# microsoft/XPretrain

Measured on NVIDIA H100. Metric: video-text pairs/sec (12f x 224^2, 32 tok), CLIP-ViP ViT-B/16 fwd+InfoNCE+bwd, higher is better.
Workload: dtype bf16

## Files before the change

### xpretrain_b200/csrc/common.cu

```cuda
#include "common.h"

#include <mutex>

#include "../../include/xpretrain_b200.h"

namespace xp {

static thread_local std::string t_error;
std::atomic<int64_t> g_launches{0};

void set_error(const std::string& msg) { t_error = msg; }
int fail(const std::string& msg) {
  t_error = msg;
  return -1;
}

int sm_count() {
  static int cached[64] = {0};
  int dev = 0;
  if (cudaGetDevice(&dev) != cudaSuccess || dev < 0 || dev >= 64) return 132;
  if (cached[dev] == 0) {
    int n = 0;
    if (cudaDeviceGetAttribute(&n, cudaDevAttrMultiProcessorCount, dev) != cudaSuccess || n <= 0) n = 132;
    cached[dev] = n;
  }
  return cached[dev];
}

typedef CUresult (*EncodeTiledFn)(CUtensorMap*, CUtensorMapDataType, cuuint32_t, void*, const cuuint64_t*,
                                  const cuuint64_t*, const cuuint32_t*, const cuuint32_t*, CUtensorMapInterleave,
                                  CUtensorMapSwizzle, CUtensorMapL2promotion, CUtensorMapFloatOOBfill);

static EncodeTiledFn encode_fn() {
  static EncodeTiledFn fn = nullptr;
  static std::once_flag once;
  std::call_once(once, [] {
    void* p = nullptr;
    cudaDriverEntryPointQueryResult q;
    if (cudaGetDriverEntryPoint("cuTensorMapEncodeTiled", &p, cudaEnableDefault, &q) == cudaSuccess &&
        q == cudaDriverEntryPointSuccess)
      fn = reinterpret_cast<EncodeTiledFn>(p);
  });
  return fn;
}

typedef CUresult (*CtxGetCurrentFn)(CUcontext*);
typedef CUresult (*CtxSetCurrentFn)(CUcontext);
typedef CUresult (*PointerGetAttributeFn)(void*, CUpointer_attribute, CUdeviceptr);

static void* driver_symbol(const char* name) {
  void* p = nullptr;
  cudaDriverEntryPointQueryResult q;
  if (cudaGetDriverEntryPoint(name, &p, cudaEnableDefault, &q) != cudaSuccess || q != cudaDriverEntryPointSuccess)
    return nullptr;
  return p;
}

int ensure_context(const void* device_ptr) {
  static thread_local bool bound = false;
  if (bound) return 0;
  static CtxGetCurrentFn get_cur = reinterpret_cast<CtxGetCurrentFn>(driver_symbol("cuCtxGetCurrent"));
  static CtxSetCurrentFn set_cur = reinterpret_cast<CtxSetCurrentFn>(driver_symbol("cuCtxSetCurrent"));
  static PointerGetAttributeFn ptr_attr =
      reinterpret_cast<PointerGetAttributeFn>(driver_symbol("cuPointerGetAttribute"));
  if (!get_cur || !set_cur || !ptr_attr)
    return fail("CUDA driver unavailable (no GPU): this library has no CPU path");
  CUcontext cur = nullptr;
  if (get_cur(&cur) == CUDA_SUCCESS && cur != nullptr) {
    bound = true;
    return 0;
  }
  if (device_ptr == nullptr) return fail("null device pointer");
  CUcontext owner = nullptr;
  if (ptr_attr(&owner, CU_POINTER_ATTRIBUTE_CONTEXT, reinterpret_cast<CUdeviceptr>(device_ptr)) == CUDA_SUCCESS &&
      owner != nullptr) {
    if (set_cur(owner) != CUDA_SUCCESS) return fail("cuCtxSetCurrent failed");
  } else {
    int ordinal = -1;
    if (ptr_attr(&ordinal, CU_POINTER_ATTRIBUTE_DEVICE_ORDINAL, reinterpret_cast<CUdeviceptr>(device_ptr)) !=
            CUDA_SUCCESS ||
        ordinal < 0)
      return fail("cannot find the CUDA device of the first pointer argument (is it a device pointer?)");
    if (cudaSetDevice(ordinal) != cudaSuccess) return fail("cudaSetDevice failed");
  }
  bound = true;
  return 0;
}

int make_tmap_bf16_2d(CUtensorMap* out, const void* base, uint64_t inner, uint64_t outer, uint64_t row_stride,
                      uint32_t box_inner, uint32_t box_outer) {
  EncodeTiledFn fn = encode_fn();
  if (!fn) return fail("cuTensorMapEncodeTiled unavailable (no CUDA driver / no GPU): this library has no CPU path");
  if ((reinterpret_cast<uintptr_t>(base) & 15) != 0) return fail("tensor map: base pointer must be 16-byte aligned");
  if ((row_stride * 2) % 16 != 0) return fail("tensor map: row stride must be a multiple of 8 bf16 elements");
  cuuint64_t dims[2] = {inner, outer};
  cuuint64_t strides[1] = {row_stride * 2};
  cuuint32_t box[2] = {box_inner, box_outer};
  cuuint32_t estr[2] = {1, 1};
  CUresult r = fn(out, CU_TENSOR_MAP_DATA_TYPE_BFLOAT16, 2, const_cast<void*>(base), dims, strides, box, estr,
                  CU_TENSOR_MAP_INTERLEAVE_NONE, CU_TENSOR_MAP_SWIZZLE_128B, CU_TENSOR_MAP_L2_PROMOTION_L2_256B,
                  CU_TENSOR_MAP_FLOAT_OOB_FILL_NONE);
  if (r != CUDA_SUCCESS) return fail("cuTensorMapEncodeTiled failed with CUresult " + std::to_string(int(r)));
  return 0;
}

int make_tmap_bf16_3d(CUtensorMap* out, const void* base, uint64_t inner, uint64_t mid, uint64_t outer,
                      uint64_t row_stride, uint64_t mid_stride, uint32_t box_inner, uint32_t box_mid) {
  EncodeTiledFn fn = encode_fn();
  if (!fn) return fail("cuTensorMapEncodeTiled unavailable (no CUDA driver / no GPU): this library has no CPU path");
  if ((reinterpret_cast<uintptr_t>(base) & 15) != 0) return fail("tensor map: base pointer must be 16-byte aligned");
  if ((row_stride * 2) % 16 != 0 || (mid_stride * 2) % 16 != 0)
    return fail("tensor map: strides must be multiples of 8 bf16 elements");
  cuuint64_t dims[3] = {inner, mid, outer};
  cuuint64_t strides[2] = {row_stride * 2, mid_stride * 2};
  cuuint32_t box[3] = {box_inner, box_mid, 1};
  cuuint32_t estr[3] = {1, 1, 1};
  CUresult r = fn(out, CU_TENSOR_MAP_DATA_TYPE_BFLOAT16, 3, const_cast<void*>(base), dims, strides, box, estr,
                  CU_TENSOR_MAP_INTERLEAVE_NONE, CU_TENSOR_MAP_SWIZZLE_128B, CU_TENSOR_MAP_L2_PROMOTION_L2_256B,
                  CU_TENSOR_MAP_FLOAT_OOB_FILL_NONE);
  if (r != CUDA_SUCCESS) return fail("cuTensorMapEncodeTiled failed with CUresult " + std::to_string(int(r)));
  return 0;
}

}

extern "C" {
int xp_version(void) { return XP_ABI_VERSION; }
const char* xp_last_error(void) { return xp::t_error.c_str(); }
int64_t xp_launch_count(void) { return xp::g_launches.load(); }
void xp_launch_count_reset(void) { xp::g_launches.store(0); }
}
```

### xpretrain_b200/csrc/common.h

```cpp
#pragma once
#include <cuda.h>
#include <cuda_runtime.h>
#include <stdint.h>

#include <atomic>
#include <string>

namespace xp {

void set_error(const std::string& msg);
int fail(const std::string& msg);
extern std::atomic<int64_t> g_launches;
inline void count_launch(int n = 1) { g_launches.fetch_add(n, std::memory_order_relaxed); }

int sm_count();

int make_tmap_bf16_2d(CUtensorMap* out, const void* base, uint64_t inner, uint64_t outer, uint64_t row_stride,
                      uint32_t box_inner, uint32_t box_outer);
int make_tmap_bf16_3d(CUtensorMap* out, const void* base, uint64_t inner, uint64_t mid, uint64_t outer,
                      uint64_t row_stride, uint64_t mid_stride, uint32_t box_inner, uint32_t box_mid);

int ensure_context(const void* device_ptr);
#define XP_ENTER(ptr)                                   \
  do {                                                  \
    if (::xp::ensure_context(ptr) != 0) return -1;      \
  } while (0)

#define XP_CHECK_CUDA(expr)                                                                         \
  do {                                                                                              \
    cudaError_t _e = (expr);                                                                        \
    if (_e != cudaSuccess) return ::xp::fail(std::string(#expr) + ": " + cudaGetErrorString(_e)); \
  } while (0)

#define XP_CHECK_LAUNCH(name)                                                                             \
  do {                                                                                                    \
    cudaError_t _e = cudaGetLastError();                                                                  \
    if (_e != cudaSuccess) return ::xp::fail(std::string(name) + " launch: " + cudaGetErrorString(_e)); \
    ::xp::count_launch();                                                                                 \
  } while (0)

}
```

### xpretrain_b200/csrc/gemm.cu

```cuda
#include "../../include/xpretrain_b200.h"
#include "common.h"
#include "ptx.cuh"
#include <cstdlib>

namespace xp {

constexpr int BM = 128;
constexpr int BK = 64;
constexpr int MMA_K = 16;
constexpr int GEMM_THREADS = 384;

struct GemmDev {
  void* c;
  const float* bias;
  const __nv_bfloat16* residual;
  __nv_bfloat16* aux;
  int M, N, K;
  long long ldc, ldr, ld_aux;
  long long c_group, c_group_stride, r_group, r_group_stride;
  int act;
  int splits;
  int scale_cols;
  float alpha, col_scale;
  uint32_t mn_lbo, mn_sbo;
};

template <int BN>
struct GemmCfg {
  static constexpr int A_BYTES = BM * BK * 2;
  static constexpr int B_BYTES = BN * BK * 2;
  static constexpr int STAGE_BYTES = A_BYTES + B_BYTES;
  static constexpr int STAGES = (BN == 256) ? 4 : 6;
  static constexpr int SMEM_BYTES = STAGES * STAGE_BYTES + 1024 + 256;
};

__device__ __forceinline__ float act_gelu_erf(float x) { return 0.5f * x * (1.f + erff(x * 0.70710678118654752f)); }
__device__ __forceinline__ float act_gelu_erf_grad(float x) {
  float cdf = 0.5f * (1.f + erff(x * 0.70710678118654752f));
  float pdf = 0.3989422804014327f * __expf(-0.5f * x * x);
  return cdf + x * pdf;
}

template <int BN, int A_MN, int B_MN, int OUT, int ACT>
__global__ void __launch_bounds__(GEMM_THREADS, 1)
gemm_kernel(const __grid_constant__ CUtensorMap tmA, const __grid_constant__ CUtensorMap tmB, const GemmDev p) {
  using Cfg = GemmCfg<BN>;
  constexpr int STAGES = Cfg::STAGES;
  constexpr bool PINGPONG = BN == 128;
  constexpr int MH = PINGPONG ? 2 : 1;
  constexpr int NH = BN / 128;
  extern __shared__ uint8_t smem_raw[];
  const uint32_t raw_addr = smem_u32(smem_raw);
  uint8_t* smem = smem_raw + (((raw_addr + 1023u) & ~1023u) - raw_addr);
  uint64_t* full_bar = reinterpret_cast<uint64_t*>(smem + STAGES * Cfg::STAGE_BYTES);
  uint64_t* empty_bar = full_bar + STAGES;

  const int wg = threadIdx.x >> 7;
  const int lane = threadIdx.x & 31;

  const int num_m = (p.M + BM - 1) / BM;
  const int num_n = (p.N + BN - 1) / BN;
  const int num_mn = num_m * num_n;
  const int total = num_mn * p.splits;
  const int kb_total = (p.K + BK - 1) / BK;
  const int kb_per = (kb_total + p.splits - 1) / p.splits;

  if (threadIdx.x == 0) {
    tma_prefetch_desc(&tmA);
    tma_prefetch_desc(&tmB);
    for (int s = 0; s < STAGES; ++s) {
      mbar_init(&full_bar[s], 1);
      mbar_init(&empty_bar[s], PINGPONG ? 1 : 2);
    }
    fence_barrier_init();
  }
  __syncthreads();

  if (wg == 0) {
    setmaxnreg_dec<40>();
    if (threadIdx.x == 0) {
      int stage = 0;
      uint32_t phase = 0;
      for (int tile = blockIdx.x; tile < total; tile += gridDim.x) {
        const int split = tile / num_mn;
        const int mn = tile - split * num_mn;
        const int m_blk = mn / num_n;
        const int n_blk = mn - m_blk * num_n;
        const int k0 = split * kb_per;
        const int k1 = min(kb_total, k0 + kb_per);
        for (int kb = k0; kb < k1; ++kb) {
          mbar_wait_nocall(&empty_bar[stage], phase ^ 1);
          uint8_t* sA = smem + stage * Cfg::STAGE_BYTES;
          uint8_t* sB = sA + Cfg::A_BYTES;
          mbar_arrive_expect_tx(&full_bar[stage], Cfg::STAGE_BYTES);
          if (A_MN) {
#pragma unroll
            for (int i = 0; i < BM / 64; ++i)
              tma_load_2d(sA + i * (BK * 128), &tmA, &full_bar[stage], m_blk * BM + i * 64, kb * BK);
          } else {
            tma_load_2d(sA, &tmA, &full_bar[stage], kb * BK, m_blk * BM);
          }
          if (B_MN) {
#pragma unroll
            for (int i = 0; i < BN / 64; ++i)
              tma_load_2d(sB + i * (BK * 128), &tmB, &full_bar[stage], n_blk * BN + i * 64, kb * BK);
          } else {
            tma_load_2d(sB, &tmB, &full_bar[stage], kb * BK, n_blk * BN);
          }
          if (++stage == STAGES) {
            stage = 0;
            phase ^= 1;
          }
        }
      }
    }
  } else {
    setmaxnreg_inc<232>();
    const int cw = wg - 1;
    const int wq = (threadIdx.x >> 5) & 3;
    constexpr int act = ACT;
    const int N = p.N, scale_cols = p.scale_cols;
    const float alpha = p.alpha, col_scale = p.col_scale;
    __nv_bfloat16* const aux_p = p.aux;
    constexpr bool need_aux_in = (ACT == XP_ACT_DQUICK_GELU || ACT == XP_ACT_DGELU_ERF);
    const __nv_bfloat16* const xin_p = need_aux_in ? p.aux : p.residual;
    constexpr uint32_t A_OFF = 64 * 128;
    const int cta_tiles = (total - blockIdx.x + gridDim.x - 1) / gridDim.x;
    int stage = 0;
    uint32_t phase = 0;
    int local = 0;
    for (int tile = blockIdx.x; tile < total; tile += gridDim.x, ++local) {
      const int split = tile / num_mn;
      const int mn = tile - split * num_mn;
      const int m_blk = mn / num_n;
      const int n_blk = mn - m_blk * num_n;
      const int k0 = split * kb_per;
      const int k1 = min(kb_total, k0 + kb_per);
      if (PINGPONG && (local & 1) != cw) {
        const int next = stage + max(0, k1 - k0);
        phase ^= (next / STAGES) & 1;
        stage = next % STAGES;
        continue;
      }
      if (PINGPONG && local > 0) named_bar_sync(1 + cw, 256);
      const bool pass_turn = PINGPONG && local + 1 < cta_tiles;
      if (k0 >= k1) {
        if (pass_turn) named_bar_arrive(2 - cw, 256);
        continue;
      }
      float acc[MH * NH][64];
#pragma unroll
      for (int q = 0; q < MH * NH; ++q)
#pragma unroll
        for (int i = 0; i < 64; ++i) acc[q][i] = 0.f;
      int prev_stage = -1;
      for (int kb = k0; kb < k1; ++kb) {
        mbar_wait_nocall(&full_bar[stage], phase);
        const uint32_t sA = smem_u32(smem + stage * Cfg::STAGE_BYTES) + (PINGPONG ? 0 : cw * A_OFF);
        const uint32_t sB = smem_u32(smem + stage * Cfg::STAGE_BYTES) + Cfg::A_BYTES;
#pragma unroll
        for (int q = 0; q < MH * NH; ++q) wgmma_fence_regs(acc[q]);
        wgmma_fence();
#pragma unroll
        for (int j = 0; j < BK / MMA_K; ++j) {
#pragma unroll
          for (int mh = 0; mh < MH; ++mh) {
            const uint32_t am = sA + mh * A_OFF;
            const uint64_t adesc = A_MN ? make_smem_desc_sw128(am + j * (MMA_K * 128), p.mn_lbo, p.mn_sbo)
                                        : make_smem_desc_sw128(am + j * (MMA_K * 2), 16, 1024);
#pragma unroll
            for (int h = 0; h < NH; ++h) {
              const uint32_t bh = sB + h * (128 * 128);
              const uint64_t bdesc = B_MN ? make_smem_desc_sw128(bh + j * (MMA_K * 128), p.mn_lbo, p.mn_sbo)
                                          : make_smem_desc_sw128(bh + j * (MMA_K * 2), 16, 1024);
              wgmma_m64n128k16_bf16<A_MN, B_MN>(acc[mh * NH + h], adesc, bdesc);
            }
          }
        }
        wgmma_commit();
#pragma unroll
        for (int q = 0; q < MH * NH; ++q) wgmma_fence_regs(acc[q]);
        wgmma_wait<1>();
        if (prev_stage >= 0 && (threadIdx.x & 127) == 0) mbar_arrive(&empty_bar[prev_stage]);
        prev_stage = stage;
        if (++stage == STAGES) {
          stage = 0;
          phase ^= 1;
        }
      }
      if (pass_turn) named_bar_arrive(2 - cw, 256);
      const auto load_bias = [&](float2(&b)[16], int h) {
#pragma unroll
        for (int i = 0; i < 16; ++i) {
          const int n = n_blk * BN + h * 128 + i * 8 + (lane & 3) * 2;
          b[i] = make_float2(0.f, 0.f);
          if (p.bias != nullptr && split == 0 && n < N) b[i] = __ldg(reinterpret_cast<const float2*>(p.bias + n));
        }
      };
      constexpr bool bias_once = PINGPONG && !need_aux_in;
      float2 bias_tile[16];
      if (bias_once) load_bias(bias_tile, 0);
      wgmma_wait<0>();
#pragma unroll
      for (int q = 0; q < MH * NH; ++q) wgmma_fence_regs(acc[q]);
      if ((threadIdx.x & 127) == 0) mbar_arrive(&empty_bar[prev_stage]);

      const auto apply = [&](float& v0, float& v1, int n, uint32_t xg) -> uint32_t {
        if (n < scale_cols) {
          v0 *= col_scale;
          v1 *= col_scale;
        }
        uint32_t pre = 0;
        if (act == XP_ACT_QUICK_GELU) {
          pre = pack_bf16(v0, v1);
          v0 = quick_gelu(v0);
          v1 = quick_gelu(v1);
        } else if (act == XP_ACT_DQUICK_GELU) {
          v0 *= quick_gelu_grad(bf16_lo(xg));
          v1 *= quick_gelu_grad(bf16_hi(xg));
        } else if (act == XP_ACT_GELU_ERF) {
          pre = pack_bf16(v0, v1);
          v0 = act_gelu_erf(v0);
          v1 = act_gelu_erf(v1);
        } else if (act == XP_ACT_DGELU_ERF) {
          v0 *= act_gelu_erf_grad(bf16_lo(xg));
          v1 *= act_gelu_erf_grad(bf16_hi(xg));
        } else if (xin_p != nullptr) {
          v0 += bf16_lo(xg);
          v1 += bf16_hi(xg);
        }
        return pre;
      };
      constexpr bool save_pre = (ACT == XP_ACT_QUICK_GELU || ACT == XP_ACT_GELU_ERF);
      const int quad = lane & 3;
#pragma unroll
      for (int mh = 0; mh < MH; ++mh) {
        const int row_base = m_blk * BM + (PINGPONG ? mh : cw) * 64 + wq * 16 + (lane >> 2);
#pragma unroll
        for (int rr = 0; rr < 2; ++rr) {
          const int row = row_base + rr * 8;
          const bool row_ok = row < p.M;
          const long long c_off = p.c_group > 0 ? (row / p.c_group) * p.c_group_stride + (row % p.c_group) * p.ldc
                                                : static_cast<long long>(row) * p.ldc;
          const long long x_off = need_aux_in ? static_cast<long long>(row) * p.ld_aux
                                              : (p.r_group > 0 ? (row / p.r_group) * p.r_group_stride + (row % p.r_group) * p.ldr
                                                               : static_cast<long long>(row) * p.ldr);
          const long long a_off = static_cast<long long>(row) * p.ld_aux;
#pragma unroll
          for (int h = 0; h < NH; ++h) {
            const float* const a = acc[mh * NH + h];
            const int n_h = n_blk * BN + h * 128;
            float2 bias2[16];
            if (bias_once) {
#pragma unroll
              for (int i = 0; i < 16; ++i) bias2[i] = bias_tile[i];
            } else {
              load_bias(bias2, h);
            }
            if (OUT == XP_OUT_BF16) {
              uint32_t xin[4][4];
#pragma unroll
              for (int k = 0; k < 4; ++k) {
                const int n8 = n_h + (4 * k + quad) * 8;
                uint4 v = make_uint4(0u, 0u, 0u, 0u);
                if (xin_p != nullptr && row_ok && n8 < N) v = *reinterpret_cast<const uint4*>(xin_p + x_off + n8);
                xin[k][0] = v.x;
                xin[k][1] = v.y;
                xin[k][2] = v.z;
                xin[k][3] = v.w;
                if (xin_p != nullptr) quad_transpose(xin[k]);
              }
#pragma unroll
              for (int k = 0; k < 4; ++k) {
                uint32_t out[4], pre[4];
#pragma unroll
                for (int j = 0; j < 4; ++j) {
                  const int i = 4 * k + j;
                  float v0 = fmaf(a[4 * i + 2 * rr], alpha, bias2[i].x);
                  float v1 = fmaf(a[4 * i + 2 * rr + 1], alpha, bias2[i].y);
                  pre[j] = apply(v0, v1, n_h + i * 8 + quad * 2, xin[k][j]);
                  out[j] = pack_bf16(v0, v1);
                }
                const int n8 = n_h + (4 * k + quad) * 8;
                quad_transpose(out);
                if (row_ok && n8 < N)
                  *reinterpret_cast<uint4*>(static_cast<__nv_bfloat16*>(p.c) + c_off + n8) =
                      make_uint4(out[0], out[1], out[2], out[3]);
                if (save_pre && aux_p != nullptr) {
                  quad_transpose(pre);
                  if (row_ok && n8 < N)
                    *reinterpret_cast<uint4*>(aux_p + a_off + n8) = make_uint4(pre[0], pre[1], pre[2], pre[3]);
                }
              }
            } else if (row_ok) {
              uint32_t xin[16];
#pragma unroll
              for (int i = 0; i < 16; ++i) {
                const int n = n_h + i * 8 + quad * 2;
                xin[i] = 0;
                if (xin_p != nullptr && n < N) xin[i] = *reinterpret_cast<const uint32_t*>(xin_p + x_off + n);
              }
#pragma unroll
              for (int i = 0; i < 16; ++i) {
                const int n = n_h + i * 8 + quad * 2;
                if (n >= N) continue;
                float v0 = fmaf(a[4 * i + 2 * rr], alpha, bias2[i].x);
                float v1 = fmaf(a[4 * i + 2 * rr + 1], alpha, bias2[i].y);
                apply(v0, v1, n, xin[i]);
                if (OUT == XP_OUT_F32) {
                  *reinterpret_cast<float2*>(static_cast<float*>(p.c) + c_off + n) = make_float2(v0, v1);
                } else {
                  asm volatile("red.global.add.v2.f32 [%0], {%1, %2};" ::"l"(static_cast<float*>(p.c) + c_off + n),
                               "f"(v0), "f"(v1)
                               : "memory");
                }
              }
            }
          }
        }
      }
    }
  }
}

template <int BN, int A_MN, int B_MN, int OUT, int ACT>
static int launch_gemm(const CUtensorMap& tmA, const CUtensorMap& tmB, const GemmDev& dev, int grid, cudaStream_t stream) {
  using Cfg = GemmCfg<BN>;
  auto kern = gemm_kernel<BN, A_MN, B_MN, OUT, ACT>;
  static bool attr_set = false;
  if (!attr_set) {
    XP_CHECK_CUDA(cudaFuncSetAttribute(kern, cudaFuncAttributeMaxDynamicSharedMemorySize, Cfg::SMEM_BYTES));
    attr_set = true;
  }
  kern<<<grid, GEMM_THREADS, Cfg::SMEM_BYTES, stream>>>(tmA, tmB, dev);
  XP_CHECK_LAUNCH("gemm_kernel");
  return 0;
}

template <int BN, int OUT, int ACT>
static int dispatch_layout(const XpGemm* g, const CUtensorMap& tmA, const CUtensorMap& tmB, const GemmDev& dev,
                           int grid, cudaStream_t stream) {
  if (g->a_layout == 0 && g->b_layout == 0) return launch_gemm<BN, 0, 0, OUT, ACT>(tmA, tmB, dev, grid, stream);
  if (g->a_layout == 0 && g->b_layout == 1) return launch_gemm<BN, 0, 1, OUT, ACT>(tmA, tmB, dev, grid, stream);
  if (g->a_layout == 1 && g->b_layout == 1) return launch_gemm<BN, 1, 1, OUT, ACT>(tmA, tmB, dev, grid, stream);
  if (g->a_layout == 1 && g->b_layout == 0) return launch_gemm<BN, 1, 0, OUT, ACT>(tmA, tmB, dev, grid, stream);
  return fail("xp_gemm: a_layout/b_layout must be 0 or 1");
}

template <int BN>
static int dispatch_act_bf16(const XpGemm* g, const CUtensorMap& tmA, const CUtensorMap& tmB, const GemmDev& dev, int grid,
                             cudaStream_t stream) {
  switch (g->act) {
    case XP_ACT_NONE: return dispatch_layout<BN, XP_OUT_BF16, XP_ACT_NONE>(g, tmA, tmB, dev, grid, stream);
    case XP_ACT_QUICK_GELU: return dispatch_layout<BN, XP_OUT_BF16, XP_ACT_QUICK_GELU>(g, tmA, tmB, dev, grid, stream);
    case XP_ACT_DQUICK_GELU: return dispatch_layout<BN, XP_OUT_BF16, XP_ACT_DQUICK_GELU>(g, tmA, tmB, dev, grid, stream);
    case XP_ACT_GELU_ERF: return dispatch_layout<BN, XP_OUT_BF16, XP_ACT_GELU_ERF>(g, tmA, tmB, dev, grid, stream);
    case XP_ACT_DGELU_ERF: return dispatch_layout<BN, XP_OUT_BF16, XP_ACT_DGELU_ERF>(g, tmA, tmB, dev, grid, stream);
  }
  return fail("xp_gemm: bad act");
}

template <int BN>
static int dispatch_out(const XpGemm* g, const CUtensorMap& tmA, const CUtensorMap& tmB, const GemmDev& dev, int grid,
                        cudaStream_t stream) {
  switch (g->out) {
    case XP_OUT_BF16: return dispatch_act_bf16<BN>(g, tmA, tmB, dev, grid, stream);
    case XP_OUT_F32: return dispatch_layout<BN, XP_OUT_F32, XP_ACT_NONE>(g, tmA, tmB, dev, grid, stream);
    case XP_OUT_F32_ATOMIC: return dispatch_layout<BN, XP_OUT_F32_ATOMIC, XP_ACT_NONE>(g, tmA, tmB, dev, grid, stream);
  }
  return fail("xp_gemm: bad out mode");
}

static int g_dbg_mn_lbo = 0, g_dbg_mn_sbo = 0;
}

extern "C" void xp_debug_gemm_mn_desc(int lbo, int sbo) {
  xp::g_dbg_mn_lbo = lbo;
  xp::g_dbg_mn_sbo = sbo;
}

extern "C" int xp_gemm(const XpGemm* g, void* stream_v) {
  using namespace xp;
  if (!g) return fail("xp_gemm: null args");
  cudaStream_t stream = static_cast<cudaStream_t>(stream_v);
  if (g->M <= 0 || g->N <= 0 || g->K <= 0) return fail("xp_gemm: M, N, K must be positive");
  if (g->N % 8 != 0) return fail("xp_gemm: N must be a multiple of 8");
  if (!g->a || !g->b || !g->c) return fail("xp_gemm: null operand");
  XP_ENTER(g->a);
  const int splits = g->splits <= 0 ? 1 : g->splits;
  if (splits > 1 && g->out != XP_OUT_F32_ATOMIC) return fail("xp_gemm: split-K requires XP_OUT_F32_ATOMIC");
  if ((g->act == XP_ACT_DQUICK_GELU || g->act == XP_ACT_DGELU_ERF) && !g->aux)
    return fail("xp_gemm: dGELU epilogue needs aux (the forward pre-activation)");
  if (g->act != XP_ACT_NONE && g->out != XP_OUT_BF16) return fail("xp_gemm: activation epilogues need a bf16 output");
  if (g->act != XP_ACT_NONE && g->residual)
    return fail("xp_gemm: a residual add cannot be combined with an activation epilogue");
  if (g->aux && g->c_group > 0) return fail("xp_gemm: aux cannot be combined with grouped rows (c_group > 0)");
  if (g->scale_cols < 0 || g->scale_cols % 2) return fail("xp_gemm: scale_cols must be even and non-negative");
  const int elem_c = g->out == XP_OUT_BF16 ? 2 : 4;
  if ((reinterpret_cast<uintptr_t>(g->c) & 15) || (g->ldc * elem_c) % 16)
    return fail("xp_gemm: C must be 16-byte aligned with a 16-byte multiple row pitch");
  if (g->bias && (reinterpret_cast<uintptr_t>(g->bias) & 15)) return fail("xp_gemm: bias must be 16-byte aligned");
  if (g->residual && ((reinterpret_cast<uintptr_t>(g->residual) & 15) || (g->ldr % 8)))
    return fail("xp_gemm: residual must be 16-byte aligned, ldr % 8 == 0");
  if (g->aux && ((reinterpret_cast<uintptr_t>(g->aux) & 15) || (g->ld_aux % 8)))
    return fail("xp_gemm: aux must be 16-byte aligned, ld_aux % 8 == 0");
  if ((g->c_group > 0 && g->c_group_stride % 8) || (g->r_group > 0 && g->r_group_stride % 8))
    return fail("xp_gemm: c_group_stride / r_group_stride must be multiples of 8 elements");

  const int nsm = sm_count();
  const int num_m = static_cast<int>((g->M + BM - 1) / BM);
  int bn = g->block_n;
  if (bn == 0) {
    const long long tiles256 = static_cast<long long>(num_m) * ((g->N + 255) / 256) * splits;
    const long long kb_split = ((g->K + BK - 1) / BK + splits - 1) / splits;
    const bool short_k_fwd = g->b_layout == 0 && kb_split <= 16;
    bn = (g->N >= 256 && tiles256 >= nsm && !short_k_fwd) ? 256 : 128;
  }
  if (bn != 128 && bn != 256) return fail("xp_gemm: block_n must be 0, 128 or 256");
  if (g->cta_pair < 0 || g->cta_pair > 1) return fail("xp_gemm: cta_pair must be 0 or 1 (no CTA pairs on sm_90)");
  const long long total = static_cast<long long>(num_m) * ((g->N + bn - 1) / bn) * splits;
  int grid = g->max_ctas > 0 ? g->max_ctas : nsm;
  if (grid < 1) grid = 1;
  if (grid > total) grid = static_cast<int>(total);

  CUtensorMap tmA, tmB;
  int rc;
  if (g->a_layout == 0)
    rc = make_tmap_bf16_2d(&tmA, g->a, g->K, g->M, g->lda, BK, BM);
  else
    rc = make_tmap_bf16_2d(&tmA, g->a, g->M, g->K, g->lda, 64, BK);
  if (rc) return rc;
  if (g->b_layout == 0)
    rc = make_tmap_bf16_2d(&tmB, g->b, g->K, g->N, g->ldb, BK, bn);
  else
    rc = make_tmap_bf16_2d(&tmB, g->b, g->N, g->K, g->ldb, 64, BK);
  if (rc) return rc;

  GemmDev dev;
  dev.c = g->c;
  dev.bias = g->bias;
  dev.residual = static_cast<const __nv_bfloat16*>(g->residual);
  dev.aux = static_cast<__nv_bfloat16*>(g->aux);
  dev.M = static_cast<int>(g->M);
  dev.N = static_cast<int>(g->N);
  dev.K = static_cast<int>(g->K);
  dev.ldc = g->ldc;
  dev.ldr = g->ldr;
  dev.ld_aux = g->ld_aux;
  dev.c_group = g->c_group;
  dev.c_group_stride = g->c_group_stride;
  dev.r_group = g->r_group;
  dev.r_group_stride = g->r_group_stride;
  dev.act = g->act;
  dev.splits = splits;
  dev.scale_cols = g->scale_cols;
  dev.alpha = g->alpha;
  dev.col_scale = g->col_scale;
  dev.mn_lbo = g_dbg_mn_lbo ? g_dbg_mn_lbo : BK * 128;
  dev.mn_sbo = g_dbg_mn_sbo ? g_dbg_mn_sbo : 1024;

  return bn == 256 ? dispatch_out<256>(g, tmA, tmB, dev, grid, stream)
                   : dispatch_out<128>(g, tmA, tmB, dev, grid, stream);
}
```

Before: 292.0.

## TMA-prefetch GELU-backward aux tile into shared memory during mainloop

For BN=256 GEMMs with a GELU-derivative epilogue, the producer warp now loads the pre-activation aux tile into shared memory via a dedicated TMA descriptor partway through the K loop. The epilogue then reads it from smem instead of issuing scattered global loads, hiding that latency behind the mainloop. To make room, pipeline stages drop from 4 to 3 for these kernels, and extra mbarriers coordinate reuse of the aux buffer across tiles. Fewer stages could reduce mainloop overlap, and the smem read path skips the row/column bounds checks the global path had.

```diff
diff --git a/xpretrain_b200/csrc/common.cu b/xpretrain_b200/csrc/common.cu
--- a/xpretrain_b200/csrc/common.cu
+++ b/xpretrain_b200/csrc/common.cu
@@ -88,7 +88,7 @@
 }
 
 int make_tmap_bf16_2d(CUtensorMap* out, const void* base, uint64_t inner, uint64_t outer, uint64_t row_stride,
-                      uint32_t box_inner, uint32_t box_outer) {
+                      uint32_t box_inner, uint32_t box_outer, CUtensorMapSwizzle swizzle) {
   EncodeTiledFn fn = encode_fn();
   if (!fn) return fail("cuTensorMapEncodeTiled unavailable (no CUDA driver / no GPU): this library has no CPU path");
   if ((reinterpret_cast<uintptr_t>(base) & 15) != 0) return fail("tensor map: base pointer must be 16-byte aligned");
@@ -98,7 +98,7 @@
   cuuint32_t box[2] = {box_inner, box_outer};
   cuuint32_t estr[2] = {1, 1};
   CUresult r = fn(out, CU_TENSOR_MAP_DATA_TYPE_BFLOAT16, 2, const_cast<void*>(base), dims, strides, box, estr,
-                  CU_TENSOR_MAP_INTERLEAVE_NONE, CU_TENSOR_MAP_SWIZZLE_128B, CU_TENSOR_MAP_L2_PROMOTION_L2_256B,
+                  CU_TENSOR_MAP_INTERLEAVE_NONE, swizzle, CU_TENSOR_MAP_L2_PROMOTION_L2_256B,
                   CU_TENSOR_MAP_FLOAT_OOB_FILL_NONE);
   if (r != CUDA_SUCCESS) return fail("cuTensorMapEncodeTiled failed with CUresult " + std::to_string(int(r)));
   return 0;
diff --git a/xpretrain_b200/csrc/common.h b/xpretrain_b200/csrc/common.h
--- a/xpretrain_b200/csrc/common.h
+++ b/xpretrain_b200/csrc/common.h
@@ -16,7 +16,8 @@
 int sm_count();
 
 int make_tmap_bf16_2d(CUtensorMap* out, const void* base, uint64_t inner, uint64_t outer, uint64_t row_stride,
-                      uint32_t box_inner, uint32_t box_outer);
+                      uint32_t box_inner, uint32_t box_outer,
+                      CUtensorMapSwizzle swizzle = CU_TENSOR_MAP_SWIZZLE_128B);
 int make_tmap_bf16_3d(CUtensorMap* out, const void* base, uint64_t inner, uint64_t mid, uint64_t outer,
                       uint64_t row_stride, uint64_t mid_stride, uint32_t box_inner, uint32_t box_mid);
 
diff --git a/xpretrain_b200/csrc/gemm.cu b/xpretrain_b200/csrc/gemm.cu
--- a/xpretrain_b200/csrc/gemm.cu
+++ b/xpretrain_b200/csrc/gemm.cu
@@ -25,13 +25,18 @@
   uint32_t mn_lbo, mn_sbo;
 };
 
-template <int BN>
+template <int BN, int ACT>
 struct GemmCfg {
+  static constexpr bool AUX_SMEM = BN == 256 && (ACT == XP_ACT_DQUICK_GELU || ACT == XP_ACT_DGELU_ERF);
   static constexpr int A_BYTES = BM * BK * 2;
   static constexpr int B_BYTES = BN * BK * 2;
   static constexpr int STAGE_BYTES = A_BYTES + B_BYTES;
-  static constexpr int STAGES = (BN == 256) ? 4 : 6;
-  static constexpr int SMEM_BYTES = STAGES * STAGE_BYTES + 1024 + 256;
+  static constexpr int STAGES = BN == 256 ? (AUX_SMEM ? 3 : 4) : 6;
+  static constexpr int AUX_BOX_COLS = 32;
+  static constexpr int AUX_BOX_BYTES = BM * AUX_BOX_COLS * 2;
+  static constexpr int AUX_BYTES = AUX_SMEM ? BM * BN * 2 : 0;
+  static constexpr int SMEM_BYTES = STAGES * STAGE_BYTES + AUX_BYTES + 1024 + 256;
+  static_assert(SMEM_BYTES <= 227 * 1024, "shared memory per CTA");
 };
 
 __device__ __forceinline__ float act_gelu_erf(float x) { return 0.5f * x * (1.f + erff(x * 0.70710678118654752f)); }
@@ -43,8 +48,10 @@
 
 template <int BN, int A_MN, int B_MN, int OUT, int ACT>
 __global__ void __launch_bounds__(GEMM_THREADS, 1)
-gemm_kernel(const __grid_constant__ CUtensorMap tmA, const __grid_constant__ CUtensorMap tmB, const GemmDev p) {
-  using Cfg = GemmCfg<BN>;
+gemm_kernel(const __grid_constant__ CUtensorMap tmA, const __grid_constant__ CUtensorMap tmB,
+            const __grid_constant__ CUtensorMap tmX, const GemmDev p) {
+  using Cfg = GemmCfg<BN, ACT>;
+  constexpr bool AUX_SMEM = Cfg::AUX_SMEM;
   constexpr int STAGES = Cfg::STAGES;
   constexpr bool PINGPONG = BN == 128;
   constexpr int MH = PINGPONG ? 2 : 1;
@@ -52,8 +59,11 @@
   extern __shared__ uint8_t smem_raw[];
   const uint32_t raw_addr = smem_u32(smem_raw);
   uint8_t* smem = smem_raw + (((raw_addr + 1023u) & ~1023u) - raw_addr);
-  uint64_t* full_bar = reinterpret_cast<uint64_t*>(smem + STAGES * Cfg::STAGE_BYTES);
+  uint8_t* const aux_smem = smem + STAGES * Cfg::STAGE_BYTES;
+  uint64_t* full_bar = reinterpret_cast<uint64_t*>(aux_smem + Cfg::AUX_BYTES);
   uint64_t* empty_bar = full_bar + STAGES;
+  uint64_t* aux_full = empty_bar + STAGES;
+  uint64_t* aux_empty = aux_full + 1;
 
   const int wg = threadIdx.x >> 7;
   const int lane = threadIdx.x & 31;
@@ -72,6 +82,11 @@
       mbar_init(&full_bar[s], 1);
       mbar_init(&empty_bar[s], PINGPONG ? 1 : 2);
     }
+    if (AUX_SMEM) {
+      tma_prefetch_desc(&tmX);
+      mbar_init(aux_full, 1);
+      mbar_init(aux_empty, 8);
+    }
     fence_barrier_init();
   }
   __syncthreads();
@@ -80,7 +95,7 @@
     setmaxnreg_dec<40>();
     if (threadIdx.x == 0) {
       int stage = 0;
-      uint32_t phase = 0;
+      uint32_t phase = 0, aux_phase = 0;
       for (int tile = blockIdx.x; tile < total; tile += gridDim.x) {
         const int split = tile / num_mn;
         const int mn = tile - split * num_mn;
@@ -88,6 +103,7 @@
         const int n_blk = mn - m_blk * num_n;
         const int k0 = split * kb_per;
         const int k1 = min(kb_total, k0 + kb_per);
+        const int kb_aux = min(k1 - 1, k0 + STAGES - 1);
         for (int kb = k0; kb < k1; ++kb) {
           mbar_wait_nocall(&empty_bar[stage], phase ^ 1);
           uint8_t* sA = smem + stage * Cfg::STAGE_BYTES;
@@ -106,6 +122,15 @@
               tma_load_2d(sB + i * (BK * 128), &tmB, &full_bar[stage], n_blk * BN + i * 64, kb * BK);
           } else {
             tma_load_2d(sB, &tmB, &full_bar[stage], kb * BK, n_blk * BN);
+          }
+          if (AUX_SMEM && kb == kb_aux) {
+            mbar_wait_nocall(aux_empty, aux_phase ^ 1);
+            mbar_arrive_expect_tx(aux_full, Cfg::AUX_BYTES);
+#pragma unroll
+            for (int j = 0; j < BN / Cfg::AUX_BOX_COLS; ++j)
+              tma_load_2d(aux_smem + j * Cfg::AUX_BOX_BYTES, &tmX, aux_full, n_blk * BN + j * Cfg::AUX_BOX_COLS,
+                          m_blk * BM);
+            aux_phase ^= 1;
           }
           if (++stage == STAGES) {
             stage = 0;
@@ -127,7 +152,7 @@
     constexpr uint32_t A_OFF = 64 * 128;
     const int cta_tiles = (total - blockIdx.x + gridDim.x - 1) / gridDim.x;
     int stage = 0;
-    uint32_t phase = 0;
+    uint32_t phase = 0, aux_phase = 0;
     int local = 0;
     for (int tile = blockIdx.x; tile < total; tile += gridDim.x, ++local) {
       const int split = tile / num_mn;
@@ -204,6 +229,7 @@
 #pragma unroll
       for (int q = 0; q < MH * NH; ++q) wgmma_fence_regs(acc[q]);
       if ((threadIdx.x & 127) == 0) mbar_arrive(&empty_bar[prev_stage]);
+      if (AUX_SMEM) mbar_wait_nocall(aux_full, aux_phase);
 
       const auto apply = [&](float& v0, float& v1, int n, uint32_t xg) -> uint32_t {
         if (n < scale_cols) {
@@ -263,7 +289,13 @@
               for (int k = 0; k < 4; ++k) {
                 const int n8 = n_h + (4 * k + quad) * 8;
                 uint4 v = make_uint4(0u, 0u, 0u, 0u);
-                if (xin_p != nullptr && row_ok && n8 < N) v = *reinterpret_cast<const uint4*>(xin_p + x_off + n8);
+                if (AUX_SMEM) {
+                  const int r = cw * 64 + wq * 16 + (lane >> 2) + rr * 8;
+                  v = *reinterpret_cast<const uint4*>(aux_smem + (h * 4 + k) * Cfg::AUX_BOX_BYTES +
+                                                      r * (Cfg::AUX_BOX_COLS * 2) + quad * 16);
+                } else if (xin_p != nullptr && row_ok && n8 < N) {
+                  v = *reinterpret_cast<const uint4*>(xin_p + x_off + n8);
+                }
                 xin[k][0] = v.x;
                 xin[k][1] = v.y;
                 xin[k][2] = v.z;
@@ -319,54 +351,60 @@
           }
         }
       }
+      if (AUX_SMEM) {
+        __syncwarp();
+        if (lane == 0) mbar_arrive(aux_empty);
+        aux_phase ^= 1;
+      }
     }
   }
 }
 
 template <int BN, int A_MN, int B_MN, int OUT, int ACT>
-static int launch_gemm(const CUtensorMap& tmA, const CUtensorMap& tmB, const GemmDev& dev, int grid, cudaStream_t stream) {
-  using Cfg = GemmCfg<BN>;
+static int launch_gemm(const CUtensorMap& tmA, const CUtensorMap& tmB, const CUtensorMap& tmX, const GemmDev& dev,
+                       int grid, cudaStream_t stream) {
+  using Cfg = GemmCfg<BN, ACT>;
   auto kern = gemm_kernel<BN, A_MN, B_MN, OUT, ACT>;
   static bool attr_set = false;
   if (!attr_set) {
     XP_CHECK_CUDA(cudaFuncSetAttribute(kern, cudaFuncAttributeMaxDynamicSharedMemorySize, Cfg::SMEM_BYTES));
     attr_set = true;
   }
-  kern<<<grid, GEMM_THREADS, Cfg::SMEM_BYTES, stream>>>(tmA, tmB, dev);
+  kern<<<grid, GEMM_THREADS, Cfg::SMEM_BYTES, stream>>>(tmA, tmB, tmX, dev);
   XP_CHECK_LAUNCH("gemm_kernel");
   return 0;
 }
 
 template <int BN, int OUT, int ACT>
-static int dispatch_layout(const XpGemm* g, const CUtensorMap& tmA, const CUtensorMap& tmB, const GemmDev& dev,
-                           int grid, cudaStream_t stream) {
-  if (g->a_layout == 0 && g->b_layout == 0) return launch_gemm<BN, 0, 0, OUT, ACT>(tmA, tmB, dev, grid, stream);
-  if (g->a_layout == 0 && g->b_layout == 1) return launch_gemm<BN, 0, 1, OUT, ACT>(tmA, tmB, dev, grid, stream);
-  if (g->a_layout == 1 && g->b_layout == 1) return launch_gemm<BN, 1, 1, OUT, ACT>(tmA, tmB, dev, grid, stream);
-  if (g->a_layout == 1 && g->b_layout == 0) return launch_gemm<BN, 1, 0, OUT, ACT>(tmA, tmB, dev, grid, stream);
+static int dispatch_layout(const XpGemm* g, const CUtensorMap& tmA, const CUtensorMap& tmB, const CUtensorMap& tmX,
+                           const GemmDev& dev, int grid, cudaStream_t stream) {
+  if (g->a_layout == 0 && g->b_layout == 0) return launch_gemm<BN, 0, 0, OUT, ACT>(tmA, tmB, tmX, dev, grid, stream);
+  if (g->a_layout == 0 && g->b_layout == 1) return launch_gemm<BN, 0, 1, OUT, ACT>(tmA, tmB, tmX, dev, grid, stream);
+  if (g->a_layout == 1 && g->b_layout == 1) return launch_gemm<BN, 1, 1, OUT, ACT>(tmA, tmB, tmX, dev, grid, stream);
+  if (g->a_layout == 1 && g->b_layout == 0) return launch_gemm<BN, 1, 0, OUT, ACT>(tmA, tmB, tmX, dev, grid, stream);
   return fail("xp_gemm: a_layout/b_layout must be 0 or 1");
 }
 
 template <int BN>
-static int dispatch_act_bf16(const XpGemm* g, const CUtensorMap& tmA, const CUtensorMap& tmB, const GemmDev& dev, int grid,
-                             cudaStream_t stream) {
+static int dispatch_act_bf16(const XpGemm* g, const CUtensorMap& tmA, const CUtensorMap& tmB, const CUtensorMap& tmX,
+                             const GemmDev& dev, int grid, cudaStream_t stream) {
   switch (g->act) {
-    case XP_ACT_NONE: return dispatch_layout<BN, XP_OUT_BF16, XP_ACT_NONE>(g, tmA, tmB, dev, grid, stream);
-    case XP_ACT_QUICK_GELU: return dispatch_layout<BN, XP_OUT_BF16, XP_ACT_QUICK_GELU>(g, tmA, tmB, dev, grid, stream);
-    case XP_ACT_DQUICK_GELU: return dispatch_layout<BN, XP_OUT_BF16, XP_ACT_DQUICK_GELU>(g, tmA, tmB, dev, grid, stream);
-    case XP_ACT_GELU_ERF: return dispatch_layout<BN, XP_OUT_BF16, XP_ACT_GELU_ERF>(g, tmA, tmB, dev, grid, stream);
-    case XP_ACT_DGELU_ERF: return dispatch_layout<BN, XP_OUT_BF16, XP_ACT_DGELU_ERF>(g, tmA, tmB, dev, grid, stream);
+    case XP_ACT_NONE: return dispatch_layout<BN, XP_OUT_BF16, XP_ACT_NONE>(g, tmA, tmB, tmX, dev, grid, stream);
+    case XP_ACT_QUICK_GELU: return dispatch_layout<BN, XP_OUT_BF16, XP_ACT_QUICK_GELU>(g, tmA, tmB, tmX, dev, grid, stream);
+    case XP_ACT_DQUICK_GELU: return dispatch_layout<BN, XP_OUT_BF16, XP_ACT_DQUICK_GELU>(g, tmA, tmB, tmX, dev, grid, stream);
+    case XP_ACT_GELU_ERF: return dispatch_layout<BN, XP_OUT_BF16, XP_ACT_GELU_ERF>(g, tmA, tmB, tmX, dev, grid, stream);
+    case XP_ACT_DGELU_ERF: return dispatch_layout<BN, XP_OUT_BF16, XP_ACT_DGELU_ERF>(g, tmA, tmB, tmX, dev, grid, stream);
   }
   return fail("xp_gemm: bad act");
 }
 
 template <int BN>
-static int dispatch_out(const XpGemm* g, const CUtensorMap& tmA, const CUtensorMap& tmB, const GemmDev& dev, int grid,
-                        cudaStream_t stream) {
+static int dispatch_out(const XpGemm* g, const CUtensorMap& tmA, const CUtensorMap& tmB, const CUtensorMap& tmX,
+                        const GemmDev& dev, int grid, cudaStream_t stream) {
   switch (g->out) {
-    case XP_OUT_BF16: return dispatch_act_bf16<BN>(g, tmA, tmB, dev, grid, stream);
-    case XP_OUT_F32: return dispatch_layout<BN, XP_OUT_F32, XP_ACT_NONE>(g, tmA, tmB, dev, grid, stream);
-    case XP_OUT_F32_ATOMIC: return dispatch_layout<BN, XP_OUT_F32_ATOMIC, XP_ACT_NONE>(g, tmA, tmB, dev, grid, stream);
+    case XP_OUT_BF16: return dispatch_act_bf16<BN>(g, tmA, tmB, tmX, dev, grid, stream);
+    case XP_OUT_F32: return dispatch_layout<BN, XP_OUT_F32, XP_ACT_NONE>(g, tmA, tmB, tmX, dev, grid, stream);
+    case XP_OUT_F32_ATOMIC: return dispatch_layout<BN, XP_OUT_F32_ATOMIC, XP_ACT_NONE>(g, tmA, tmB, tmX, dev, grid, stream);
   }
   return fail("xp_gemm: bad out mode");
 }
@@ -435,6 +473,11 @@
   else
     rc = make_tmap_bf16_2d(&tmB, g->b, g->N, g->K, g->ldb, 64, BK);
   if (rc) return rc;
+  CUtensorMap tmX = {};
+  if (bn == 256 && (g->act == XP_ACT_DQUICK_GELU || g->act == XP_ACT_DGELU_ERF)) {
+    rc = make_tmap_bf16_2d(&tmX, g->aux, g->N, g->M, g->ld_aux, 32, BM, CU_TENSOR_MAP_SWIZZLE_NONE);
+    if (rc) return rc;
+  }
 
   GemmDev dev;
   dev.c = g->c;
@@ -459,6 +502,6 @@
   dev.mn_lbo = g_dbg_mn_lbo ? g_dbg_mn_lbo : BK * 128;
   dev.mn_sbo = g_dbg_mn_sbo ? g_dbg_mn_sbo : 1024;
 
-  return bn == 256 ? dispatch_out<256>(g, tmA, tmB, dev, grid, stream)
-                   : dispatch_out<128>(g, tmA, tmB, dev, grid, stream);
-}
+  return bn == 256 ? dispatch_out<256>(g, tmA, tmB, tmX, dev, grid, stream)
+                   : dispatch_out<128>(g, tmA, tmB, tmX, dev, grid, stream);
+}
```

Result: no change. 294.0 (median of 6 runs) (+0.7%).
